# Minys233/GCN-BMP

Hardware: AMD Instinct MI355X
Metric: drug-pairs/sec fwd+bwd, binary-DDI GGNN d=128 (higher is better)
Workload: dtype f32; 1 GPU; C2: full binary DDI set (544 drugs, 147696 pairs), GGNN 4-step d=128 tied + Nie co-attention (head 8, tanh) + MLP(32,16), fwd+bwd+Adam, 1024 pairs/GPU/step, every molecule instance encoded; the 144 batches of one epoch resident in HBM, cycled; layout=per-instance packed layout, whole 128-row tiles, pairs_per_gpu=1024, global_batch=1024, parallelism=dp1

## Files before the change

gcn-bmp_amd/csrc/bmp_fused.hip:

```cpp
#include <type_traits>
#include <string.h>
#include "bmp_kernels.h"

#include "bmp_tile.h"

template <int D, bool FIRST, bool VAR, bool SAVE>
__global__ __launch_bounds__(512) void k_ggnn_step_fwd(StepArgs a) {
    constexpr int LD = D + 4;
    constexpr int NCB = D / 32, NRW = 8 / NCB, RB = 4 / NRW;
    extern __shared__ __attribute__((aligned(16))) float lds[];
    float* Hs = lds;
    float* As = lds + FZ_R * LD;
    float* wds = As + FZ_R * LD;
    int* rptr = (int*)(wds + FZ_R * 4);
    int* ecol = rptr + 132;
    float* evalv = (float*)(ecol + FZ_ECAP);
    int* sy = (int*)(evalv + FZ_ECAP);

    const int tid = threadIdx.x, lane = tid & 63, w = tid >> 6;
    const int grp = w >> 2;
    GrpSync gs{sy + grp, 0};
    if (tid < FZ_NSYNC) sy[tid] = 0;
    if (grp == 0) __builtin_amdgcn_s_setprio(2);
    const int wc = w % NCB, wr = w / NCB;
    const int l31 = lane & 31, hi = lane >> 5;
    FZ_TILE_SETUP();
    if (VAR && a.tile_stride > nrows) {
        const int e = row0 + a.tile_stride;
        fz_clear_rows<512>(a.hout, D, row0 + nrows, e, tid);
        fz_clear_rows<512>(a.m, D, row0 + nrows, e, tid);
        fz_clear_rows<512>(a.rz, 2 * D, row0 + nrows, e, tid);
        fz_clear_rows<512>(a.c, D, row0 + nrows, e, tid);
    }
    const int col = wc * 32 + l31;
    const int wrow0 = wr * RB * 32;
    const int lrow = wrow0 + 4 * hi;
    const int rot = (tile * 8) % D;
    const float* Hw = Hs + (wrow0 + l31) * LD + 4 * hi;
    const float* Aw = As + (wrow0 + l31) * LD + 4 * hi;
    float* Hl = Hs + lrow * LD + col;
    float* Al = As + lrow * LD + col;
#define LOFF(rb, reg) (((rb) * 32 + ((reg) & 3) + 8 * ((reg) >> 2)) * LD)

    constexpr bool save = SAVE;
    for (int idx = tid; idx < nrows * (D / 4); idx += 512) {
        const int r = idx / (D / 4), c4 = idx % (D / 4);
        *(f32x4*)(Hs + r * LD + 4 * c4) = *(const f32x4*)(a.h + (size_t)(row0 + r) * D + 4 * c4);
    }
    const bool csr_lds = stage_csr(a.ptr, a.col, a.val, row0, rptr, ecol, evalv, nrows);
    __syncthreads();
    if (!grp_live) return;
    const RowOrder ro = FZ_ROW_ORDER();
    const int bi = wr & 1;

    auto step = [&](auto first_c, const float* WTs, const float* bEs, const float* ATs, const float* bvs, float* om, float* orz,
                    float* oc, float* oh) {
        constexpr bool FST = decltype(first_c)::value;
        int tmask = 0;
        f32x16 acc_m[1][RB];
        zero_acc(acc_m[0]);
        for (int e = 0; e < 4; ++e) {
            const float* const Bp[1] = {WTs + (size_t)(e * D + 4 * hi) * D + 4 * col};
            const int ldw[1] = {D};
            BPre<1> pre;
            tile_b_prefetch<1>(pre, Bp, ldw, D, rot);
            float wd;
            FZ_GATHER(Hs, As, e, &wd);
            if ((tid & 3) == 0) wds[(tid >> 2) * 4 + e] = wd;
            if (e == 0 && (tid & 3) == 0 && tmask) __hip_atomic_fetch_or(sy + 2 + grp, tmask, __ATOMIC_RELAXED, __HIP_MEMORY_SCOPE_WORKGROUP);
            grp_sync(gs);
            const int any = (__hip_atomic_load(sy + 2 + grp, __ATOMIC_RELAXED, __HIP_MEMORY_SCOPE_WORKGROUP) >> e) & 1;
            if (any) tile_mma_msg<VAR, 1, RB>(nrb, e, ro.nbr, bi, acc_m, Aw, LD, Bp, ldw, D, rot, &pre);
            FZ_GSYNC();
        }
        constexpr int NG = FST ? 2 : 3;
        int ldwg[NG];
    #pragma unroll
        for (int g = 0; g < NG; ++g) ldwg[g] = 3 * D;
        const float* const base_h = ATs + (size_t)(4 * hi) * 3 * D + 4 * col + (FST ? 4 * D : 0);
        const float* const base_m = ATs + (size_t)(D + 4 * hi) * 3 * D + 4 * col + (FST ? 4 * D : 0);
        const float* Bh[NG]; const float* Bm[NG];
    #pragma unroll
        for (int g = 0; g < NG; ++g) { Bh[g] = base_h + 4 * D * g; Bm[g] = base_m + 4 * D * g; }
        BPre<NG> pre_h;
        tile_b_prefetch<NG>(pre_h, (const float* const (&)[NG])Bh, (const int (&)[NG])ldwg, D, rot);
        {
            const AccBuf mo = acc_buf<D>(om, row0, 0, col);
            float be[4];
    #pragma unroll
            for (int e = 0; e < 4; ++e) be[e] = bEs[e * D + col];
            FZ_FOR_ACC {
                const int tp = lrow + rb * 32 + (reg & 3) + 8 * (reg >> 2);
                const int r = (tp & 64) + ro.perm[tp];
                const f32x4 wd4 = *(const f32x4*)(wds + r * 4);
                const float v = __builtin_fmaf(wd4[3], be[3], __builtin_fmaf(wd4[2], be[2], __builtin_fmaf(wd4[1], be[1],
                                               __builtin_fmaf(wd4[0], be[0], acc_m[0][rb][reg]))));
                As[r * LD + col] = v;
                if (save) __builtin_amdgcn_raw_buffer_store_b32(__builtin_bit_cast(unsigned, v), mo.rs, mo.vo + r * D * 4, 0, 0);
            }
        }
        FZ_GSYNC();

        f32x16 acc_g[3][RB];
        zero_acc(acc_g[0]); zero_acc(acc_g[1]); zero_acc(acc_g[2]);
        {
            f32x16 gg[NG][RB];
    #pragma unroll
            for (int g = 0; g < NG; ++g) zero_acc(gg[g]);
            BPre<NG> pre_m;
            tile_b_prefetch<NG>(pre_m, (const float* const (&)[NG])Bm, (const int (&)[NG])ldwg, D, rot);
            tile_mma_n<VAR, NG, RB>(nrb, gg, Hw, LD, (const float* const (&)[NG])Bh, (const int (&)[NG])ldwg, D, rot, &pre_h);
            tile_mma_n<VAR, NG, RB>(nrb, gg, Aw, LD, (const float* const (&)[NG])Bm, (const int (&)[NG])ldwg, D, rot, &pre_m);
    #pragma unroll
            for (int g = 0; g < NG; ++g)
    #pragma unroll
                for (int rb = 0; rb < RB; ++rb) acc_g[g + (FST ? 1 : 0)][rb] = gg[g][rb];
        }
        const float br = bvs[col], bz = bvs[D + col], bcn = bvs[2 * D + col];
        {
            const AccBuf rzo = acc_buf<2 * D>(orz, row0, lrow, col);
            FZ_FOR_ACC {
                const float zv = bmp_sigmoid(acc_g[1][rb][reg] + bz);
                acc_g[1][rb][reg] = zv;
                if (save) acc_st<2 * D>(rzo, rb, reg, zv, D);
                if (!FST) {
                    const float rv = bmp_sigmoid(acc_g[0][rb][reg] + br);
                    acc_g[0][rb][reg] = rv;
                    if (save) acc_st<2 * D>(rzo, rb, reg, rv, 0);
                }
            }
        }
        if (!FST) {
            const float* const Bu[1] = {a.UcT + (size_t)(4 * hi) * D + 4 * col};
            const int ldu[1] = {D};
            BPre<1> pre_u;
            tile_b_prefetch<1>(pre_u, Bu, ldu, D, rot);
            FZ_GSYNC();
            FZ_FOR_ACC { Al[LOFF(rb, reg)] = acc_g[0][rb][reg] * Hl[LOFF(rb, reg)]; }
            FZ_GSYNC();
            f32x16 gc[1][RB];
    #pragma unroll
            for (int rb = 0; rb < RB; ++rb) gc[0][rb] = acc_g[2][rb];
            tile_mma_n<VAR, 1, RB>(nrb, gc, Aw, LD, Bu, ldu, D, rot, &pre_u);
    #pragma unroll
            for (int rb = 0; rb < RB; ++rb) acc_g[2][rb] = gc[0][rb];
        }
        {
            const AccBuf co = acc_buf<D>(oc, row0, lrow, col);
            const AccBuf ho = acc_buf<D>(oh, row0, lrow, col);
            FZ_FOR_ACC {
                const float cv = bmp_tanh(acc_g[2][rb][reg] + bcn);
                const float zv = acc_g[1][rb][reg];
                float hn = zv * cv;
                if (!FST) hn = __builtin_fmaf(1.f - zv, Hl[LOFF(rb, reg)], hn);
                if (save) acc_st<D>(co, rb, reg, cv);
                acc_st<D>(ho, rb, reg, hn);
            }
        }
    };
    step(std::integral_constant<bool, FIRST>{}, a.WT, a.bE, a.AT, a.b, a.m, a.rz, a.c, a.hout);
}

template <int D, bool FIRST, bool VAR>
__global__ __launch_bounds__(512) void k_ggnn_step_bwd(StepArgs a) {
    constexpr int LD = D + 4;
    constexpr int NCB = D / 32, NRW = 8 / NCB, RB = 4 / NRW;
    constexpr int F4 = D / 4;
    constexpr int NV = D / 16;
    extern __shared__ __attribute__((aligned(16))) float lds[];
    float* Xs = lds;
    float* Ys = lds + FZ_R * LD;
    int* rptr = (int*)(Ys + FZ_R * LD + FZ_R * 4);
    int* ecol = rptr + 132;
    float* evalv = (float*)(ecol + FZ_ECAP);
    int* sy = (int*)(evalv + FZ_ECAP);

    const int tid = threadIdx.x, lane = tid & 63, w = tid >> 6;
    const int grp = w >> 2;
    GrpSync gs{sy + grp, 0};
    int tmask = 0;
    if (tid < FZ_NSYNC) sy[tid] = 0;
    if (grp == 0) __builtin_amdgcn_s_setprio(2);
    const int wc = w % NCB, wr = w / NCB;
    const int l31 = lane & 31, hi = lane >> 5;
    FZ_TILE_SETUP();
    if (VAR && a.tile_stride > nrows) {
        const int e = row0 + a.tile_stride;
        fz_clear_rows<512>(a.dh, D, row0 + nrows, e, tid);
        fz_clear_rows<512>(a.gda, 7 * D, row0 + nrows, e, tid);
    }
    const int col = wc * 32 + l31;
    const int wrow0 = wr * RB * 32;
    const int lrow = wrow0 + 4 * hi;
    const int rot = (tile * 8) % D;
    const float* Xw = Xs + (wrow0 + l31) * LD + 4 * hi;
    const float* Yw = Ys + (wrow0 + l31) * LD + 4 * hi;
    float* Xl = Xs + lrow * LD + col;
    float* Yl = Ys + lrow * LD + col;
    constexpr bool first = FIRST;
    const int tg = tid & 255;
#define RM_ROW(v) (grp * 64 + ((v) * 256 + tg) / F4)
#define RM_C4(v) (((v) * 256 + tg) % F4)
#define RM_LDS(T, v) (*(f32x4*)((T) + RM_ROW(v) * LD + 4 * RM_C4(v)))
#define RM_LIVE(v) (!VAR || grp * 64 + (v) * (256 / F4) < nrows)
    const AccBuf b_g = rm_buf<D, D>(a.dhout, row0, grp, tg), b_c = rm_buf<D, D>(a.c, row0, grp, tg);
    const AccBuf b_h = rm_buf<D, D>(a.h, row0, grp, tg), b_rz = rm_buf<D, 2 * D>(a.rz, row0, grp, tg);
    const AccBuf b_o = rm_buf<D, 7 * D>(a.gda, row0, grp, tg), b_dh = rm_buf<D, D>(a.dh, row0, grp, tg);

    const bool csr_lds = stage_csr(a.ptr, a.col, a.val, row0, rptr, ecol, evalv, nrows);
    if (!grp_live) {
        __syncthreads();
        return;
    }

    f32x4 ex[NV];
    {
        const f32x4 one = (f32x4){1.f, 1.f, 1.f, 1.f};
        f32x4 g4[NV], z4[NV], c4[NV], h4[NV];
#pragma unroll
        for (int v = 0; v < NV; ++v) if (RM_LIVE(v)) {
            g4[v] = rm_ld<D, D>(b_g, v);
            z4[v] = rm_ld<D, 2 * D>(b_rz, v, D);
            c4[v] = rm_ld<D, D>(b_c, v);
            if (!first) h4[v] = rm_ld<D, D>(b_h, v);
        }
#pragma unroll
        for (int v = 0; v < NV; ++v) if (RM_LIVE(v)) {
            const f32x4 gz = g4[v] * z4[v];
            const f32x4 dac = gz * (one - c4[v] * c4[v]);
            f32x4 dz = gz * (one - z4[v]);
            if (first) { dz *= c4[v]; ex[v] = (f32x4){0.f, 0.f, 0.f, 0.f}; }
            else { dz *= (c4[v] - h4[v]); ex[v] = g4[v] - gz; }
            RM_LDS(Xs, v) = dac;
            RM_LDS(Ys, v) = dz;
            rm_st<D, 7 * D>(b_o, v, dac, 6 * D);
            rm_st<D, 7 * D>(b_o, v, dz, 5 * D);
        }
    }
    const float* const Ac_h = a.A + (size_t)(2 * D + 4 * hi) * 2 * D + 4 * col;
    const float* const Az_h = a.A + (size_t)(D + 4 * hi) * 2 * D + 4 * col;
    const float* const Ar_h = a.A + (size_t)(4 * hi) * 2 * D + 4 * col;
    const int ld2[2] = {2 * D, 2 * D};
    const float* const Bc[2] = {Ac_h, Ac_h + 4 * D};
    BPre<2> pre_c;
    tile_b_prefetch<2>(pre_c, Bc, ld2, D, rot);
    __syncthreads();
    const RowOrder ro = FZ_ROW_ORDER();
    const int bi = wr & 1;
    int aoff[RB];
#pragma unroll
    for (int rb = 0; rb < RB; ++rb) { const int tp = wrow0 + rb * 32 + l31; aoff[rb] = (((tp & 64) + ro.perm[tp]) - (wrow0 + l31)) * LD; }
#define FZ_ROWOF(rb, reg) ((lrow & 64) + ro.perm[lrow + (rb) * 32 + ((reg) & 3) + 8 * ((reg) >> 2)])

    f32x16 acc_x[2][RB];
    zero_acc(acc_x[0]); zero_acc(acc_x[1]);
    tile_mma_n<VAR, 2, RB>(nrb, acc_x, Xw, LD, Bc, ld2, D, rot, &pre_c, aoff);
    if (!first) {
        f32x16 acc_d[1][RB];
        zero_acc(acc_d[0]);
        {
            const float* const Bu[1] = {a.Uc + (size_t)(4 * hi) * D + 4 * col};
            const int ldu[1] = {D};
            tile_mma_n<VAR, 1, RB>(nrb, acc_d, Xw, LD, Bu, ldu, D, rot, nullptr, aoff);
        }
        FZ_GSYNC();
        FZ_FOR_ACC { Xs[FZ_ROWOF(rb, reg) * LD + col] = acc_d[0][rb][reg]; }
        f32x4 r4[NV], h4[NV];
#pragma unroll
        for (int v = 0; v < NV; ++v) if (RM_LIVE(v)) { r4[v] = rm_ld<D, 2 * D>(b_rz, v); h4[v] = rm_ld<D, D>(b_h, v); }
        FZ_GSYNC();
#pragma unroll
        for (int v = 0; v < NV; ++v) if (RM_LIVE(v)) {
            const f32x4 drh = RM_LDS(Xs, v);
            const f32x4 dr = drh * r4[v];
            const f32x4 dar = dr * h4[v] * ((f32x4){1.f, 1.f, 1.f, 1.f} - r4[v]);
            ex[v] += dr;
            RM_LDS(Xs, v) = dar;
            rm_st<D, 7 * D>(b_o, v, dar, 4 * D);
        }
        FZ_GSYNC();
        {
            const float* const Br[2] = {Ar_h, Ar_h + 4 * D};
            tile_mma_n<VAR, 2, RB>(nrb, acc_x, Xw, LD, Br, ld2, D, rot, nullptr, aoff);
        }
    }
    {
        const float* const Bz[2] = {Az_h, Az_h + 4 * D};
        tile_mma_n<VAR, 2, RB>(nrb, acc_x, Yw, LD, Bz, ld2, D, rot, nullptr, aoff);
    }
    FZ_GSYNC();
    FZ_FOR_ACC { Xs[FZ_ROWOF(rb, reg) * LD + col] = acc_x[1][rb][reg]; }
    __syncthreads();

    f32x16 acc_h[1][RB];
#pragma unroll
    for (int rb = 0; rb < RB; ++rb) acc_h[0][rb] = acc_x[0][rb];
    for (int e = 0; e < 4; ++e) {
        const float* const Bp[1] = {a.Wnat + (size_t)(4 * hi) * 4 * D + 4 * (e * D + col)};
        const int ldw[1] = {4 * D};
        BPre<1> pre;
        tile_b_prefetch<1>(pre, Bp, ldw, D, rot);
        float wd;
        const bool has_e = FZ_GATHER(Xs, Ys, e, &wd);
        if ((tid >> 2) < nrows && (has_e || !a.skip_zero_g)) {
            const int row = tid >> 2, q = tid & 3;
            const float* s = Ys + ((row & 64) + ro.inv[row]) * LD + q * (D / 4);
            float* o = a.gda + (size_t)(row0 + row) * 7 * D + e * D + q * (D / 4);
#pragma unroll
            for (int f = 0; f < D / 16; ++f) *(f32x4*)(o + 4 * f) = *(const f32x4*)(s + 4 * f);
        }
        if (e == 0 && (tid & 3) == 0 && tmask) __hip_atomic_fetch_or(sy + 2 + grp, tmask, __ATOMIC_RELAXED, __HIP_MEMORY_SCOPE_WORKGROUP);
        grp_sync(gs);
        const int any = (__hip_atomic_load(sy + 2 + grp, __ATOMIC_RELAXED, __HIP_MEMORY_SCOPE_WORKGROUP) >> e) & 1;
        if (any) tile_mma_msg<VAR, 1, RB>(nrb, e, ro.nbr, bi, acc_h, Yw, LD, Bp, ldw, D, rot, &pre);
        FZ_GSYNC();
    }
    FZ_FOR_ACC { Ys[FZ_ROWOF(rb, reg) * LD + col] = acc_h[0][rb][reg]; }
    FZ_GSYNC();
#pragma unroll
    for (int v = 0; v < NV; ++v) if (RM_LIVE(v)) rm_st<D, D>(b_dh, v, RM_LDS(Ys, v) + ex[v]);
#undef RM_LIVE
#undef RM_ROW
#undef RM_C4
#undef RM_LDS
#undef FZ_ROWOF
}

struct RelArgs {
    const int* ptr; const int* col; const float* val;
    int tile0;
    int act;
    const int* mt_row0; const int* mt_nblk;
    int mt_rows;
    const float* h;
    const float* WT;
    const float* bE;
    const float* WsT;
    const float* bs;
    float* out;
    float* wdeg;
    const float* dout; const float* y;
    const float* Wnat;
    const float* Ws;
    float* dh;
    float* gda;
    int skip_zero_g;
};

template <int D, bool VAR>
__global__ __launch_bounds__(512) void k_relgcn_layer_fwd(RelArgs a) {
    constexpr int LD = D + 4;
    constexpr int NCB = D / 32, NRW = 8 / NCB, RB = 4 / NRW;
    extern __shared__ __attribute__((aligned(16))) float lds[];
    float* Hs = lds;
    float* As = lds + FZ_R * LD;
    float* wds = As + FZ_R * LD;
    int* rptr = (int*)(wds + FZ_R * 4);
    int* ecol = rptr + 132;
    float* evalv = (float*)(ecol + FZ_ECAP);
    int* sy = (int*)(evalv + FZ_ECAP);

    const int tid = threadIdx.x, lane = tid & 63, w = tid >> 6;
    const int grp = w >> 2;
    GrpSync gs{sy + grp, 0};
    int tmask = 0;
    if (tid < FZ_NSYNC) sy[tid] = 0;
    if (grp == 0) __builtin_amdgcn_s_setprio(2);
    const int wc = w % NCB, wr = w / NCB;
    const int l31 = lane & 31, hi = lane >> 5;
    FZ_TILE_SETUP();
    const int col = wc * 32 + l31;
    const int wrow0 = wr * RB * 32;
    const int lrow = wrow0 + 4 * hi;
    const int rot = (tile * 8) % D;
    const float* Hw = Hs + (wrow0 + l31) * LD + 4 * hi;
    const float* Aw = As + (wrow0 + l31) * LD + 4 * hi;

    for (int idx = tid; idx < nrows * (D / 4); idx += 512) {
        const int r = idx / (D / 4), c4 = idx % (D / 4);
        *(f32x4*)(Hs + r * LD + 4 * c4) = *(const f32x4*)(a.h + (size_t)(row0 + r) * D + 4 * c4);
    }
    const bool csr_lds = stage_csr(a.ptr, a.col, a.val, row0, rptr, ecol, evalv, nrows);
    __syncthreads();
    if (!grp_live) return;
    const RowOrder ro = FZ_ROW_ORDER();
    const int bi = wr & 1;
    int aoff[RB];
#pragma unroll
    for (int rb = 0; rb < RB; ++rb) { const int tp = wrow0 + rb * 32 + l31; aoff[rb] = (((tp & 64) + ro.perm[tp]) - (wrow0 + l31)) * LD; }

    f32x16 acc[1][RB];
    zero_acc(acc[0]);
    const float* const Bs[1] = {a.WsT + (size_t)(4 * hi) * D + 4 * col};
    const int lds_[1] = {D};
    BPre<1> pre_s;
    for (int e = 0; e < 4; ++e) {
        const float* const Bp[1] = {a.WT + (size_t)(e * D + 4 * hi) * D + 4 * col};
        const int ldw[1] = {D};
        BPre<1> pre;
        tile_b_prefetch<1>(pre, Bp, ldw, D, rot);
        if (e == 3) tile_b_prefetch<1>(pre_s, Bs, lds_, D, rot);
        float wd;
        FZ_GATHER(Hs, As, e, &wd);
        if ((tid & 3) == 0) wds[(tid >> 2) * 4 + e] = wd;
        if (e == 0 && (tid & 3) == 0 && tmask) __hip_atomic_fetch_or(sy + 2 + grp, tmask, __ATOMIC_RELAXED, __HIP_MEMORY_SCOPE_WORKGROUP);
        grp_sync(gs);
        const int any = (__hip_atomic_load(sy + 2 + grp, __ATOMIC_RELAXED, __HIP_MEMORY_SCOPE_WORKGROUP) >> e) & 1;
        if (any) tile_mma_msg<VAR, 1, RB>(nrb, e, ro.nbr, bi, acc, Aw, LD, Bp, ldw, D, rot, &pre);
        FZ_GSYNC();
    }
    tile_mma_n<VAR, 1, RB>(nrb, acc, Hw, LD, Bs, lds_, D, rot, &pre_s, aoff);
    {
        const AccBuf oo = acc_buf<D>(a.out, row0, 0, col);
        float be[4];
#pragma unroll
        for (int e = 0; e < 4; ++e) be[e] = a.bE[e * D + col];
        const float bsv = a.bs ? a.bs[col] : 0.f;
        const int act = a.act;
        FZ_FOR_ACC {
            const int tp = lrow + rb * 32 + (reg & 3) + 8 * (reg >> 2);
            const int r = (tp & 64) + ro.perm[tp];
            const f32x4 wd4 = *(const f32x4*)(wds + r * 4);
            const float v = acc[0][rb][reg] + bsv + wd4[0] * be[0] + wd4[1] * be[1] + wd4[2] * be[2] + wd4[3] * be[3];
            __builtin_amdgcn_raw_buffer_store_b32(__builtin_bit_cast(unsigned, bmp_act(act, v)), oo.rs, oo.vo + r * D * 4, 0, 0);
        }
    }
    if (a.wdeg != nullptr && (tid & 255) < 64 && grp * 64 + (tid & 255) < nrows) {
        const int r = grp * 64 + (tid & 255);
        *(f32x4*)(a.wdeg + (size_t)(row0 + r) * 4) = *(const f32x4*)(wds + r * 4);
    }
}

template <int D, bool VAR>
__global__ __launch_bounds__(512) void k_relgcn_layer_bwd(RelArgs a) {
    constexpr int LD = D + 4;
    constexpr int NCB = D / 32, NRW = 8 / NCB, RB = 4 / NRW;
    constexpr int F4 = D / 4;
    constexpr int NV = D / 16;
    extern __shared__ __attribute__((aligned(16))) float lds[];
    float* Xs = lds;
    float* Ys = lds + FZ_R * LD;
    int* rptr = (int*)(Ys + FZ_R * LD + FZ_R * 4);
    int* ecol = rptr + 132;
    float* evalv = (float*)(ecol + FZ_ECAP);
    int* sy = (int*)(evalv + FZ_ECAP);

    const int tid = threadIdx.x, lane = tid & 63, w = tid >> 6;
    const int grp = w >> 2;
    GrpSync gs{sy + grp, 0};
    int tmask = 0;
    if (tid < FZ_NSYNC) sy[tid] = 0;
    if (grp == 0) __builtin_amdgcn_s_setprio(2);
    const int wc = w % NCB, wr = w / NCB;
    const int l31 = lane & 31, hi = lane >> 5;
    FZ_TILE_SETUP();
    const int col = wc * 32 + l31;
    const int wrow0 = wr * RB * 32;
    const int lrow = wrow0 + 4 * hi;
    const int rot = (tile * 8) % D;
    const float* Xw = Xs + (wrow0 + l31) * LD + 4 * hi;
    const float* Yw = Ys + (wrow0 + l31) * LD + 4 * hi;
    float* Yl = Ys + lrow * LD + col;
    const int tg = tid & 255;
#define RM_ROW(v) (grp * 64 + ((v) * 256 + tg) / F4)
#define RM_C4(v) (((v) * 256 + tg) % F4)
#define RM_LDS(T, v) (*(f32x4*)((T) + RM_ROW(v) * LD + 4 * RM_C4(v)))
#define RM_LIVE(v) (!VAR || grp * 64 + (v) * (256 / F4) < nrows)
    const AccBuf b_g = rm_buf<D, D>(a.dout, row0, grp, tg), b_y = rm_buf<D, D>(a.y, row0, grp, tg);
// ... 410 lines not shown
```

gcn-bmp_amd/csrc/bmp_ops.hip:

```cpp
#include <string.h>
#include "bmp_kernels.h"

static inline RGArgs rg_zero() {
    RGArgs a;
    memset(&a, 0, sizeof(a));
    return a;
}

static inline size_t max_sz(size_t a, size_t b) { return a > b ? a : b; }

__global__ void k_dact(const float* __restrict__ dout, int lddo, const float* __restrict__ out, int ldo, int act, int N,
                       int d, float* __restrict__ dpre) {
    const size_t total = (size_t)N * d;
    for (size_t idx = (size_t)blockIdx.x * blockDim.x + threadIdx.x; idx < total; idx += (size_t)gridDim.x * blockDim.x) {
        const int row = (int)(idx / d), c = (int)(idx % d);
        dpre[idx] = dout[(size_t)row * lddo + c] * bmp_dact(act, out[(size_t)row * ldo + c]);
    }
}

__global__ void k_gru_bwd_gates(const float* __restrict__ dhn, const float* __restrict__ h, const float* __restrict__ rz,
                                const float* __restrict__ c, int N, int d, int first, float* __restrict__ da,
                                float* __restrict__ dhacc) {
    const size_t total = (size_t)N * d;
    for (size_t idx = (size_t)blockIdx.x * blockDim.x + threadIdx.x; idx < total; idx += (size_t)gridDim.x * blockDim.x) {
// ... 303 lines not shown
        a.c_out = c; a.ldc = d;
        a.first = 0;
        if ((rc = bmp_launch_rowgemm(a, n_tiles, BMP_EPI_GRU_OUT, st))) return rc;
    }
    return 0;
}

extern "C" size_t bmp_gru_state_bwd_ws_floats(int n_tiles, int d) { return bmp_gru_bwd_ws_floats(n_tiles, d); }

extern "C" int bmp_gru_state_bwd(const float* dsout, const float* hd, const float* m, const float* s, const float* rz,
                                 const float* c, int n_tiles, int d, const float* A, const float* Urz, const float* Uc, float* dhd,
                                 float* dm, float* ds, float* dWT, float* dUrzT, float* dUcT, float* db, float* ws,
                                 size_t ws_floats, hipStream_t st) {
    BMP_REQUIRE(n_tiles > 0 && d > 0 && (d & 7) == 0 && ws_floats >= bmp_gru_state_bwd_ws_floats(n_tiles, d));
    BMP_REQUIRE(dsout && hd && m && s && rz && c && A && Urz && Uc && dhd && dm && ds && dWT && dUrzT && dUcT && db && ws);
    const int N = n_tiles * BMP_R;
    float* da = ws;
    float* dsacc = da + (size_t)N * 3 * d;
    float* slab = dsacc + (size_t)N * d;
    int rc;
    hipLaunchKernelGGL(k_gru_bwd_gates, dim3(ew_blocks((size_t)N * d)), dim3(256), 0, st, dsout, s, rz, c, N, d, 0, da, dsacc);
    BMP_LAUNCH_CHECK();
    {
        RGArgs a = rg_zero();
        a.s[0] = RGSrc{da + 2 * d, nullptr, Uc, 3 * d, 0, d, d};
        a.nsrc = 1; a.Nout = d;
        a.Y = da; a.ldy = 3 * d;
        a.r = rz; a.ldr = 2 * d;
        a.h = s; a.ldh = d;
        a.o1 = dsacc; a.ldo1 = d;
        if ((rc = bmp_launch_rowgemm(a, n_tiles, BMP_EPI_GRU_DRH, st))) return rc;
    }
    {
        RGArgs a = rg_zero();
        a.s[0] = RGSrc{da, nullptr, A, 3 * d, 0, 2 * d, 3 * d};
        a.nsrc = 1; a.Nout = 2 * d;
        a.Y = dhd; a.ldy = d;
        a.split = d;
        a.o1 = dm; a.ldo1 = d;
        if ((rc = bmp_launch_rowgemm(a, n_tiles, BMP_EPI_GENERIC, st))) return rc;
    }
    {
        RGArgs a = rg_zero();
        a.s[0] = RGSrc{da, nullptr, Urz, 3 * d, 0, d, 2 * d};
        a.nsrc = 1; a.Nout = d;
        a.Y = ds; a.ldy = d;
        a.add = dsacc; a.ldadd = d;
        if ((rc = bmp_launch_rowgemm(a, n_tiles, BMP_EPI_GENERIC, st))) return rc;
    }
    {
        WGArgs g{hd, nullptr, d, 0, da, 3 * d, d, 3 * d, N, dWT, 3 * d, 0, db};
        if ((rc = bmp_launch_wgrad(g, slab, st))) return rc;
        WGArgs g2{m, nullptr, d, 0, da, 3 * d, d, 3 * d, N, dWT + (size_t)d * 3 * d, 3 * d, 0};
        if ((rc = bmp_launch_wgrad(g2, slab, st))) return rc;
        WGArgs g3{s, nullptr, d, 0, da, 3 * d, d, 2 * d, N, dUrzT, 2 * d, 0};
        if ((rc = bmp_launch_wgrad(g3, slab, st))) return rc;
        WGArgs g4{rz, s, 2 * d, d, da + 2 * d, 3 * d, d, d, N, dUcT, d, 0};
        if ((rc = bmp_launch_wgrad(g4, slab, st))) return rc;
    }
    return 0;
}

extern "C" int bmp_readout_fwd(const float* h, const float* h0, int n_tiles, int d, int d0, int o, const float* WT,
                               const float* b, int act_j, const float* row_w, const int* mol_row0, const int* mol_nrows,
                               int n_mols, float* ij, float* g, hipStream_t st) {
    BMP_REQUIRE(n_tiles > 0 && d > 0 && (d & 7) == 0 && o > 0 && n_mols > 0);
    BMP_REQUIRE(h0 == nullptr || (d0 > 0 && (d0 & 7) == 0));
    RGArgs a = rg_zero();
    a.s[0] = RGSrc{h, nullptr, WT, d, 0, 2 * o, d};
    a.nsrc = 1;
    if (h0) {
        a.s[1] = RGSrc{h0, nullptr, WT + (size_t)d * 2 * o, d0, 0, 2 * o, d0};
        a.nsrc = 2;
    }
    a.Nout = 2 * o;
    a.Y = ij; a.ldy = 2 * o;
    a.bias = b;
    a.split = o;
    a.act_lo = BMP_ACT_SIGMOID; a.act_hi = act_j;
    int rc = bmp_launch_rowgemm(a, n_tiles, BMP_EPI_GENERIC, st);
    if (rc) return rc;
    hipLaunchKernelGGL(k_readout_segsum, dim3(n_mols), dim3(256), 0, st, ij, o, row_w, mol_row0, mol_nrows, g);
    BMP_LAUNCH_CHECK();
    return 0;
}

extern "C" size_t bmp_readout_bwd_ws_floats(int n_tiles, int d, int d0, int o) {
    const int N = n_tiles * BMP_R;
    size_t slab = max_sz(bmp_wgrad_ws_floats(N, d, 2 * o), d0 > 0 ? bmp_wgrad_ws_floats(N, d0, 2 * o) : 0);
    slab = max_sz(slab, bmp_colsum_ws_floats(N, 2 * o));
    return (size_t)N * 2 * o + slab;
}

extern "C" int bmp_readout_bwd(const float* dg, const float* h, const float* h0, int n_tiles, int d, int d0, int o,
                               const float* Wnat, const float* ij, int act_j, const float* row_w, const int* mol_row0,
                               const int* mol_nrows, int n_mols, float* dh, float* dh0, float* dWT, float* db,
                               int accumulate_w, float* ws, size_t ws_floats, hipStream_t st, hipStream_t st_w) {
    BMP_REQUIRE(n_tiles > 0 && d > 0 && (d & 7) == 0 && o > 0 && (o & 3) == 0 && n_mols > 0);
    if (!h0) d0 = 0;
    BMP_REQUIRE(ws_floats >= bmp_readout_bwd_ws_floats(n_tiles, d, d0, o));
    const int N = n_tiles * BMP_R;
    float* dij = ws;
    float* slab = dij + (size_t)N * 2 * o;
    hipError_t e = hipMemsetAsync(dij, 0, (size_t)N * 2 * o * sizeof(float), st);
    if (e != hipSuccess) return (int)e;
    hipLaunchKernelGGL(k_readout_bwd_rows, dim3(n_mols), dim3(256), 0, st, dg, ij, o, act_j, row_w, mol_row0, mol_nrows, dij);
    BMP_LAUNCH_CHECK();
    int rc;
    const int acc = accumulate_w ? 1 : 0;
    if (!st_w) st_w = st;
    if ((rc = bmp_fork_to(st, st_w))) return rc;
    {
        RGArgs a = rg_zero();
        a.s[0] = RGSrc{dij, nullptr, Wnat, 2 * o, 0, d + d0, 2 * o};
        a.nsrc = 1; a.Nout = d + d0;
        a.Y = dh; a.ldy = d;
        if (h0) { a.split = d; a.o1 = dh0; a.ldo1 = d0; }
        if ((rc = bmp_launch_rowgemm(a, n_tiles, BMP_EPI_GENERIC, st))) return rc;
    }
    {
        WGArgs g{h, nullptr, d, 0, dij, 2 * o, d, 2 * o, N, dWT, 2 * o, acc, db};
        if ((rc = bmp_launch_wgrad(g, slab, st_w))) return rc;
        if (h0) {
            WGArgs g2{h0, nullptr, d0, 0, dij, 2 * o, d0, 2 * o, N, dWT + (size_t)d * 2 * o, 2 * o, acc};
            if ((rc = bmp_launch_wgrad(g2, slab, st_w))) return rc;
        }
    }
    return 0;
}

extern "C" int bmp_linear_fwd(const float* X, int ldx, int n_tiles, int K, int Nout, const float* WT, int ldw,
                              const float* b, int act, float* Y, int ldy, hipStream_t st) {
    RGArgs a = rg_zero();
    a.s[0] = RGSrc{X, nullptr, WT, ldx, 0, ldw, K};
    a.nsrc = 1; a.Nout = Nout; a.Y = Y; a.ldy = ldy; a.bias = b;
    a.act_lo = a.act_hi = act;
    return bmp_launch_rowgemm(a, n_tiles, BMP_EPI_GENERIC, st);
}

extern "C" size_t bmp_wgrad_ws_floats_c(int N, int K, int Nn) {
    return max_sz(bmp_wgrad_ws_floats(N, K, Nn), bmp_colsum_ws_floats(N, Nn));
}

extern "C" int bmp_linear_wgrad(const float* X, int ldx, const float* dY, int ldy, int N, int K, int Nn, float* dWT,
                                float* db, float* ws, size_t ws_floats, hipStream_t st) {
    BMP_REQUIRE(ws_floats >= bmp_wgrad_ws_floats_c(N, K, Nn));
    WGArgs g{X, nullptr, ldx, 0, dY, ldy, K, Nn, N, dWT, Nn, 0};
    int rc = bmp_launch_wgrad(g, ws, st);
    if (rc) return rc;
    if (db) return bmp_launch_colsum(dY, ldy, N, Nn, db, 0, ws, st);
    return 0;
}

extern "C" int bmp_version(void) { return 409; }
extern "C" int bmp_tile_rows(void) { return BMP_R; }
```

gcn-bmp_amd/csrc/bmp_tile.h:

```cpp
#pragma once
#include <stdlib.h>
#include <type_traits>
#include <string.h>
#include "bmp_kernels.h"

#define FZ_R 128

struct StepArgs {
    const int* ptr; const int* col; const float* val;
    int tile0;
    int first;
    const int* mt_row0; const int* mt_nblk;
    int mt_rows;
    const float* h;
    const float* WT;
    const float* bE;
    const float* AT;
    const float* UcT;
    const float* b;
    float* m; float* rz; float* c; float* hout;
    const float* dhout;
    const float* Wnat;
    const float* A;
    const float* Uc;
    float* dh;
    float* gda;
    int skip_zero_g;
    int tile_stride;
};

template <int NT>
__device__ __forceinline__ void fz_clear_rows(float* p, int W, int r_begin, int r_end, int tid) {
    if (p == nullptr) return;
    const int w4 = W >> 2;
    f32x4* q = (f32x4*)(p + (size_t)r_begin * W);
    const int n = (r_end - r_begin) * w4;
    for (int i = tid; i < n; i += NT) q[i] = (f32x4){0.f, 0.f, 0.f, 0.f};
}

template <int NB>
struct BPre { f32x4 b0[NB], b1[NB]; };
template <int NB>
__device__ __forceinline__ void tile_b_prefetch(BPre<NB>& p, const float* const (&Bp)[NB], const int (&ldw)[NB], int K, int rot) {
    int k1 = rot + 8; if (k1 >= K) k1 -= K;
#pragma unroll
    for (int nb = 0; nb < NB; ++nb) {
        p.b0[nb] = *(const f32x4*)(Bp[nb] + (size_t)rot * ldw[nb]);
        p.b1[nb] = *(const f32x4*)(Bp[nb] + (size_t)k1 * ldw[nb]);
    }
}

template <int NB, int RB, int NRB = RB>
__device__ __forceinline__ void tile_mma(f32x16 (&acc)[NB][RB], const float* As_wave, int LD, const float* const (&Bp)[NB],
                                         const int (&ldw)[NB], int K, int rot, const BPre<NB>* pre = nullptr, const int* aoff = nullptr) {
    f32x4 b0[NB], b1[NB], b2[NB];
    int k = rot;
    int k1 = k + 8; if (k1 >= K) k1 -= K;
#pragma unroll
    for (int nb = 0; nb < NB; ++nb) {
        if (pre) { b0[nb] = pre->b0[nb]; b1[nb] = pre->b1[nb]; }
        else {
            b0[nb] = *(const f32x4*)(Bp[nb] + (size_t)k * ldw[nb]);
            b1[nb] = *(const f32x4*)(Bp[nb] + (size_t)k1 * ldw[nb]);
        }
    }
    f32x4 a0[NRB], a1[NRB];
#pragma unroll
    for (int rb = 0; rb < NRB; ++rb) a0[rb] = *(const f32x4*)(As_wave + (aoff ? aoff[rb] : rb * 32 * LD) + k);
    for (int it = 0; it < K; it += 8) {
        int k2 = k1 + 8; if (k2 >= K) k2 -= K;
#pragma unroll
        for (int nb = 0; nb < NB; ++nb) b2[nb] = *(const f32x4*)(Bp[nb] + (size_t)k2 * ldw[nb]);
#pragma unroll
        for (int rb = 0; rb < NRB; ++rb) a1[rb] = *(const f32x4*)(As_wave + (aoff ? aoff[rb] : rb * 32 * LD) + k1);
        __builtin_amdgcn_sched_barrier(0);
#pragma unroll
        for (int t = 0; t < 4; ++t)
#pragma unroll
            for (int rb = 0; rb < NRB; ++rb)
#pragma unroll
                for (int nb = 0; nb < NB; ++nb) acc[nb][rb] = bmp_mfma(a0[rb][t], b0[nb][t], acc[nb][rb]);
        __builtin_amdgcn_sched_barrier(0);
#pragma unroll
        for (int nb = 0; nb < NB; ++nb) { b0[nb] = b1[nb]; b1[nb] = b2[nb]; }
#pragma unroll
        for (int rb = 0; rb < NRB; ++rb) a0[rb] = a1[rb];
        k = k1; k1 = k2;
    }
}

template <bool VAR, int NB, int RB>
__device__ __forceinline__ void tile_mma_n(int nrb, f32x16 (&acc)[NB][RB], const float* As_wave, int LD, const float* const (&Bp)[NB],
                                           const int (&ldw)[NB], int K, int rot, const BPre<NB>* pre = nullptr, const int* aoff = nullptr) {
    if constexpr (!VAR) {
        tile_mma<NB, RB, RB>(acc, As_wave, LD, Bp, ldw, K, rot, pre, aoff);
    } else if constexpr (RB == 1) {
        if (nrb > 0) tile_mma<NB, 1, 1>(acc, As_wave, LD, Bp, ldw, K, rot, pre, aoff);
    } else {
        if (nrb == RB) tile_mma<NB, RB, RB>(acc, As_wave, LD, Bp, ldw, K, rot, pre, aoff);
        else if (nrb > 0) tile_mma<NB, RB, 1>(acc, As_wave, LD, Bp, ldw, K, rot, pre, aoff);
    }
}

template <int N>
__device__ __forceinline__ void zero_acc(f32x16 (&acc)[N]) {
#pragma unroll
    for (int i = 0; i < N; ++i)
#pragma unroll
        for (int r = 0; r < 16; ++r) acc[i][r] = 0.f;
}

template <int D>
__device__ __forceinline__ bool tile_gather(const float* src_tile, float* dst_tile, int LD, const int* ptr, const int* col,
                                            const float* val, int row0, int e, float* wsum, int* tmask, int nrows = FZ_R,
                                            const unsigned char* inv = nullptr) {
    constexpr int F = D / 16;
    const int row = threadIdx.x >> 2, q = threadIdx.x & 3;
    f32x4 acc[F];
#pragma unroll
    for (int f = 0; f < F; ++f) acc[f] = (f32x4){0.f, 0.f, 0.f, 0.f};
    float wd = 0.f;
    bool any = false;
    *wsum = 0.f;
    if (nrows < FZ_R && row >= nrows) return false;
    const int e0 = ptr[row], e1 = ptr[row + 1];
    for (int ed = e0; ed < e1; ++ed) {
        const int cv = col[ed];
        *tmask |= 1 << (cv & 3);
        if ((cv & 3) == e) {
            const float v = val[ed];
            const float* s = src_tile + ((cv >> 2) - row0) * LD + q * (D / 4);
#pragma unroll
            for (int f = 0; f < F; ++f) acc[f] += *(const f32x4*)(s + 4 * f) * v;
            wd += v;
            any = true;
        }
    }
    float* o = dst_tile + (inv ? (row & 64) + inv[row] : row) * LD + q * (D / 4);
#pragma unroll
    for (int f = 0; f < F; ++f) *(f32x4*)(o + 4 * f) = acc[f];
    *wsum = wd;
    return any;
}

#define FZ_ECAP 1024
__device__ __forceinline__ bool stage_csr(const int* ptr, const int* col, const float* val, int row0, int* rptr, int* ecol,
                                          float* evalv, int nrows = FZ_R, int nt = 512) {
    const int ebase = ptr[row0];
    const int ne = ptr[row0 + nrows] - ebase;
    if (ne > FZ_ECAP) return false;
    for (int i = threadIdx.x; i <= nrows; i += nt) rptr[i] = ptr[row0 + i] - ebase;
    for (int i = threadIdx.x; i < ne; i += nt) { ecol[i] = col[ebase + i]; evalv[i] = val[ebase + i]; }
    return true;
}
#define FZ_GATHER(srcT, dstT, e, wdp) (csr_lds ? tile_gather<D>(srcT, dstT, LD, rptr, ecol, evalv, row0, e, wdp, &tmask, nrows, ro.inv) \
                                               : tile_gather<D>(srcT, dstT, LD, a.ptr + row0, a.col, a.val, row0, e, wdp, &tmask, nrows, ro.inv))
#define FZ_ROW_ORDER() fz_row_order(sy, gs, grp, w, lane, csr_lds ? rptr : a.ptr + row0, csr_lds ? ecol : a.col, nrows)

struct GrpSync {
    int* ctr;
    int target;
};
__device__ __forceinline__ void grp_sync(GrpSync& g) {
    g.target += 4;
    __builtin_amdgcn_fence(__ATOMIC_RELEASE, "workgroup", "local");
    if ((threadIdx.x & 63) == 0) __hip_atomic_fetch_add(g.ctr, 1, __ATOMIC_RELAXED, __HIP_MEMORY_SCOPE_WORKGROUP);
    while (__hip_atomic_load(g.ctr, __ATOMIC_RELAXED, __HIP_MEMORY_SCOPE_WORKGROUP) < g.target) __builtin_amdgcn_s_sleep(1);
    __builtin_amdgcn_fence(__ATOMIC_ACQUIRE, "workgroup", "local");
}
#define FZ_NSYNC 72

#define FZ_RARE_TYPES 0x6
struct RowOrder {
    const unsigned char* inv;
    const unsigned char* perm;
    int nbr;
};
__device__ __forceinline__ RowOrder fz_row_order(int* sy, GrpSync& gs, int grp, int w, int lane, const int* ptr_local, const int* col,
                                                 int nrows) {
    unsigned char* inv = (unsigned char*)(sy + 8);
    unsigned char* perm = (unsigned char*)(sy + 40);
    if ((w & 3) == 0) {
        const int r = grp * 64 + lane;
        int m = 0;
        if (r < nrows)
            for (int ed = ptr_local[r]; ed < ptr_local[r + 1]; ++ed) m |= 1 << (col[ed] & 3);
        const bool rare = (m & FZ_RARE_TYPES) != 0;
        const unsigned long long bal = __ballot(rare), lt = (1ull << lane) - 1ull;
        const int nr = __popcll(bal);
        const int pos = rare ? __popcll(bal & lt) : nr + __popcll(~bal & lt);
        inv[r] = (unsigned char)pos;
        perm[grp * 64 + pos] = (unsigned char)lane;
        if (lane == 0) sy[4 + grp] = nr;
    }
    grp_sync(gs);
    return RowOrder{inv, perm, (sy[4 + grp] + 31) >> 5};
}
template <bool VAR, int NB, int RB>
__device__ __forceinline__ void tile_mma_msg(int nrb, int e, int nbr, int bi, f32x16 (&acc)[NB][RB], const float* As_wave, int LD,
                                             const float* const (&Bp)[NB], const int (&ldw)[NB], int K, int rot, const BPre<NB>* pre) {
    const bool rare = (FZ_RARE_TYPES >> e) & 1;
    if constexpr (RB == 1) {
        if (nrb > 0 && (!rare || bi < nbr)) tile_mma<NB, 1, 1>(acc, As_wave, LD, Bp, ldw, K, rot, pre);
    } else {
        const int nb = rare ? (nbr < nrb ? nbr : nrb) : nrb;
        if (nb >= RB) tile_mma<NB, RB, RB>(acc, As_wave, LD, Bp, ldw, K, rot, pre);
        else if (nb > 0) tile_mma<NB, RB, 1>(acc, As_wave, LD, Bp, ldw, K, rot, pre);
    }
}

struct AccBuf {
    __amdgpu_buffer_rsrc_t rs;
    int vo;
};
template <int LDC>
__device__ __forceinline__ AccBuf acc_buf(const float* base, int tile_row0, int lane_row, int col) {
    AccBuf b;
    b.rs = __builtin_amdgcn_make_buffer_rsrc((void*)(base + (size_t)tile_row0 * LDC), 0, 0x7FFFFFFF, 0x00020000);
    b.vo = (lane_row * LDC + col) * 4;
    return b;
}
template <int LDC>
__device__ __forceinline__ float acc_ld(const AccBuf& b, int rb, int reg, int coff = 0) {
    const int so = ((rb * 32 + (reg & 3) + 8 * (reg >> 2)) * LDC + coff) * 4;
    return __builtin_bit_cast(float, __builtin_amdgcn_raw_buffer_load_b32(b.rs, b.vo, so, 0));
}
template <int LDC>
__device__ __forceinline__ void acc_st(const AccBuf& b, int rb, int reg, float v, int coff = 0) {
    const int so = ((rb * 32 + (reg & 3) + 8 * (reg >> 2)) * LDC + coff) * 4;
    __builtin_amdgcn_raw_buffer_store_b32(__builtin_bit_cast(unsigned, v), b.rs, b.vo, so, 0);
}

typedef unsigned u32x4 __attribute__((ext_vector_type(4)));
template <int D, int LDP>
__device__ __forceinline__ AccBuf rm_buf(const float* base, int tile_row0, int grp, int tg) {
    AccBuf b;
    b.rs = __builtin_amdgcn_make_buffer_rsrc((void*)(base + (size_t)tile_row0 * LDP), 0, 0x7FFFFFFF, 0x00020000);
    b.vo = ((grp * 64 + tg / (D / 4)) * LDP + 4 * (tg % (D / 4))) * 4;
    return b;
}
template <int D, int LDP>
__device__ __forceinline__ f32x4 rm_ld(const AccBuf& b, int v, int coff = 0) {
    const int so = (v * (1024 / D) * LDP + coff) * 4;
    return __builtin_bit_cast(f32x4, __builtin_amdgcn_raw_buffer_load_b128(b.rs, b.vo, so, 0));
}
template <int D, int LDP>
__device__ __forceinline__ void rm_st(const AccBuf& b, int v, f32x4 x, int coff = 0) {
    const int so = (v * (1024 / D) * LDP + coff) * 4;
    __builtin_amdgcn_raw_buffer_store_b128(__builtin_bit_cast(u32x4, x), b.rs, b.vo + so, 0, 0);
}

#define FZ_FOR_ACC _Pragma("unroll") for (int rb = 0; rb < RB; ++rb) if (rb < nrb) _Pragma("unroll") for (int reg = 0; reg < 16; ++reg)

template <int D>
__device__ __forceinline__ int fz_live(int nblk, int wr) {
    constexpr int NCB = D / 32, NRW = 8 / NCB, RB = 4 / NRW;
    const int live = nblk - wr * RB;
    return live < 0 ? 0 : (live > RB ? RB : live);
}
#define FZ_TILE_SETUP()                                                          \
    const int tile = blockIdx.x + a.tile0;                                      \
    const int row0 = VAR ? a.mt_row0[tile] : tile * FZ_R;                       \
    const int nblk = VAR ? a.mt_nblk[tile] : 4;                                 \
    const int nrows = VAR ? nblk * 32 : FZ_R;                                   \
    const int nrb = VAR ? fz_live<D>(nblk, wr) : RB;                            \
    const bool grp_live = VAR ? nblk > 2 * grp : true

#define FZ_GSYNC() grp_sync(gs)
```

Measured before the change: 403,300 pairs/s.

## Interleave gda gradient stores with message MFMA loop and spill ex through dh

The per-edge-type copy of the gathered gradient tile from LDS to global gda now happens inside the MFMA K-loop. A side lambda issues one buffer store per iteration, and sched_group_barrier interleaves those stores with the MFMAs instead of running them as a separate phase before the matmul. To save registers, the ex accumulator is no longer held across the edge-type loop: the partial dh is written to global early and reloaded before the final sum. This aims to hide store latency and lower VGPR pressure, but it adds an extra global write and read of dh and depends on the compiler honoring the scheduling hints.

New measurement: 405,800 pairs/s, median of 6. No clear change (+0.6%).

```diff
diff --git a/gcn-bmp_amd/csrc/bmp_fused.hip b/gcn-bmp_amd/csrc/bmp_fused.hip
--- a/gcn-bmp_amd/csrc/bmp_fused.hip
+++ b/gcn-bmp_amd/csrc/bmp_fused.hip
@@ -161,6 +161,19 @@
     step(std::integral_constant<bool, FIRST>{}, a.WT, a.bE, a.AT, a.b, a.m, a.rz, a.c, a.hout);
 }
 
+template <bool VAR>
+__device__ __forceinline__ f32x4 fz_ex_plus_dr(f32x4 ex, f32x4 drh, f32x4 r, f32x4 dr) {
+    f32x4 o;
+    if constexpr (VAR) {
+#pragma unroll
+        for (int t = 0; t < 4; ++t) o[t] = __builtin_fmaf(drh[t], r[t], ex[t]);
+    } else {
+#pragma clang fp contract(off)
+        o = ex + dr;
+    }
+    return o;
+}
+
 template <int D, bool FIRST, bool VAR>
 __global__ __launch_bounds__(512) void k_ggnn_step_bwd(StepArgs a) {
     constexpr int LD = D + 4;
@@ -229,7 +242,7 @@
             const f32x4 gz = g4[v] * z4[v];
             const f32x4 dac = gz * (one - c4[v] * c4[v]);
             f32x4 dz = gz * (one - z4[v]);
-            if (first) { dz *= c4[v]; ex[v] = (f32x4){0.f, 0.f, 0.f, 0.f}; }
+            if (first) dz *= c4[v];
             else { dz *= (c4[v] - h4[v]); ex[v] = g4[v] - gz; }
             RM_LDS(Xs, v) = dac;
             RM_LDS(Ys, v) = dz;
@@ -274,7 +287,7 @@
             const f32x4 drh = RM_LDS(Xs, v);
             const f32x4 dr = drh * r4[v];
             const f32x4 dar = dr * h4[v] * ((f32x4){1.f, 1.f, 1.f, 1.f} - r4[v]);
-            ex[v] += dr;
+            rm_st<D, D>(b_dh, v, fz_ex_plus_dr<VAR>(ex[v], drh, r4[v], dr));
             RM_LDS(Xs, v) = dar;
             rm_st<D, 7 * D>(b_o, v, dar, 4 * D);
         }
@@ -292,6 +305,7 @@
     FZ_FOR_ACC { Xs[FZ_ROWOF(rb, reg) * LD + col] = acc_x[1][rb][reg]; }
     __syncthreads();
 
+    const __amdgpu_buffer_rsrc_t g_rs = __builtin_amdgcn_make_buffer_rsrc((void*)(a.gda + (size_t)row0 * 7 * D), 0, nrows * 7 * D * 4, 0x00020000);
     f32x16 acc_h[1][RB];
 #pragma unroll
     for (int rb = 0; rb < RB; ++rb) acc_h[0][rb] = acc_x[0][rb];
@@ -302,18 +316,35 @@
         tile_b_prefetch<1>(pre, Bp, ldw, D, rot);
         float wd;
         const bool has_e = FZ_GATHER(Xs, Ys, e, &wd);
-        if ((tid >> 2) < nrows && (has_e || !a.skip_zero_g)) {
-            const int row = tid >> 2, q = tid & 3;
-            const float* s = Ys + ((row & 64) + ro.inv[row]) * LD + q * (D / 4);
-            float* o = a.gda + (size_t)(row0 + row) * 7 * D + e * D + q * (D / 4);
-#pragma unroll
-            for (int f = 0; f < D / 16; ++f) *(f32x4*)(o + 4 * f) = *(const f32x4*)(s + 4 * f);
-        }
+        const bool g_st = (tid >> 2) < nrows && (has_e || !a.skip_zero_g);
+        const int g_row = tid >> 2, g_q = tid & 3;
+        const float* g_s = Ys + ((g_row & 64) + ro.inv[g_row]) * LD + g_q * (D / 4);
         if (e == 0 && (tid & 3) == 0 && tmask) __hip_atomic_fetch_or(sy + 2 + grp, tmask, __ATOMIC_RELAXED, __HIP_MEMORY_SCOPE_WORKGROUP);
         grp_sync(gs);
         const int any = (__hip_atomic_load(sy + 2 + grp, __ATOMIC_RELAXED, __HIP_MEMORY_SCOPE_WORKGROUP) >> e) & 1;
-        if (any) tile_mma_msg<VAR, 1, RB>(nrb, e, ro.nbr, bi, acc_h, Yw, LD, Bp, ldw, D, rot, &pre);
+        bool stored = false;
+        if (any) {
+            const int g_vo = g_st ? (g_row * 7 * D + e * D + g_q * (D / 4)) * 4 : (int)0x80000000u;
+            f32x4 g_cur = *(const f32x4*)g_s;
+            auto g_side = [&](int i, auto) {
+                if (i < D / 16) {
+                    __builtin_amdgcn_raw_buffer_store_b128(__builtin_bit_cast(u32x4, g_cur), g_rs, g_vo + 16 * i, 0, 0);
+                    if (i + 1 < D / 16) g_cur = *(const f32x4*)(g_s + 4 * (i + 1));
+                }
+            };
+            stored = tile_mma_msg_side<VAR, D, 2, 1, RB>(nrb, e, ro.nbr, bi, acc_h, Yw, LD, Bp, ldw, rot, &pre, g_side);
+        }
+        if (!stored && g_st) {
+            float* o = a.gda + (size_t)(row0 + g_row) * 7 * D + e * D + g_q * (D / 4);
+#pragma unroll
+            for (int f = 0; f < D / 16; ++f) *(f32x4*)(o + 4 * f) = *(const f32x4*)(g_s + 4 * f);
+        }
         FZ_GSYNC();
+    }
+#pragma unroll
+    for (int v = 0; v < NV; ++v) {
+        ex[v] = (f32x4){0.f, 0.f, 0.f, 0.f};
+        if (!first && RM_LIVE(v)) ex[v] = rm_ld<D, D>(b_dh, v);
     }
     FZ_FOR_ACC { Ys[FZ_ROWOF(rb, reg) * LD + col] = acc_h[0][rb][reg]; }
     FZ_GSYNC();
diff --git a/gcn-bmp_amd/csrc/bmp_ops.hip b/gcn-bmp_amd/csrc/bmp_ops.hip
--- a/gcn-bmp_amd/csrc/bmp_ops.hip
+++ b/gcn-bmp_amd/csrc/bmp_ops.hip
@@ -479,5 +479,5 @@
     return 0;
 }
 
-extern "C" int bmp_version(void) { return 409; }
+extern "C" int bmp_version(void) { return 410; }
 extern "C" int bmp_tile_rows(void) { return BMP_R; }
diff --git a/gcn-bmp_amd/csrc/bmp_tile.h b/gcn-bmp_amd/csrc/bmp_tile.h
--- a/gcn-bmp_amd/csrc/bmp_tile.h
+++ b/gcn-bmp_amd/csrc/bmp_tile.h
@@ -89,6 +89,57 @@
     }
 }
 
+#define FZ_SG_MFMA 0x008
+#define FZ_SG_VMEM_READ 0x020
+#define FZ_SG_DS_READ 0x100
+#define FZ_SG_SIDE (0x002 | 0x004 | 0x040 | 0x080 | 0x400)
+template <int NB, int RB, int NRB, int K, int SPM, class Side>
+__device__ __forceinline__ void tile_mma_side(f32x16 (&acc)[NB][RB], const float* As_wave, int LD, const float* const (&Bp)[NB],
+                                              const int (&ldw)[NB], int rot, const BPre<NB>* pre, const int* aoff, Side& side) {
+    f32x4 b0[NB], b1[NB], b2[NB];
+    int k = rot;
+    int k1 = k + 8; if (k1 >= K) k1 -= K;
+#pragma unroll
+    for (int nb = 0; nb < NB; ++nb) {
+        if (pre) { b0[nb] = pre->b0[nb]; b1[nb] = pre->b1[nb]; }
+        else {
+            b0[nb] = *(const f32x4*)(Bp[nb] + (size_t)k * ldw[nb]);
+            b1[nb] = *(const f32x4*)(Bp[nb] + (size_t)k1 * ldw[nb]);
+        }
+    }
+    f32x4 a0[NRB], a1[NRB];
+#pragma unroll
+    for (int rb = 0; rb < NRB; ++rb) a0[rb] = *(const f32x4*)(As_wave + (aoff ? aoff[rb] : rb * 32 * LD) + k);
+    __builtin_amdgcn_sched_barrier(0);
+#pragma unroll
+    for (int i = 0; i < K / 8; ++i) {
+        int k2 = k1 + 8; if (k2 >= K) k2 -= K;
+#pragma unroll
+        for (int nb = 0; nb < NB; ++nb) b2[nb] = *(const f32x4*)(Bp[nb] + (size_t)k2 * ldw[nb]);
+#pragma unroll
+        for (int rb = 0; rb < NRB; ++rb) a1[rb] = *(const f32x4*)(As_wave + (aoff ? aoff[rb] : rb * 32 * LD) + k1);
+        side(i, std::integral_constant<int, NRB>{});
+#pragma unroll
+        for (int t = 0; t < 4; ++t)
+#pragma unroll
+            for (int rb = 0; rb < NRB; ++rb)
+#pragma unroll
+                for (int nb = 0; nb < NB; ++nb) acc[nb][rb] = bmp_mfma(a0[rb][t], b0[nb][t], acc[nb][rb]);
+        __builtin_amdgcn_sched_group_barrier(FZ_SG_VMEM_READ, NB, 0);
+        __builtin_amdgcn_sched_group_barrier(FZ_SG_DS_READ, NRB, 0);
+#pragma unroll
+        for (int q = 0; q < 4 * NRB * NB; ++q) {
+            __builtin_amdgcn_sched_group_barrier(FZ_SG_MFMA, 1, 0);
+            __builtin_amdgcn_sched_group_barrier(FZ_SG_SIDE, SPM, 0);
+        }
+        __builtin_amdgcn_sched_barrier(0);
+#pragma unroll
+        for (int nb = 0; nb < NB; ++nb) { b0[nb] = b1[nb]; b1[nb] = b2[nb]; }
+#pragma unroll
+        for (int rb = 0; rb < NRB; ++rb) a0[rb] = a1[rb];
+        k = k1; k1 = k2;
+    }
+}
 template <bool VAR, int NB, int RB>
 __device__ __forceinline__ void tile_mma_n(int nrb, f32x16 (&acc)[NB][RB], const float* As_wave, int LD, const float* const (&Bp)[NB],
                                            const int (&ldw)[NB], int K, int rot, const BPre<NB>* pre = nullptr, const int* aoff = nullptr) {
@@ -209,6 +260,20 @@
     }
 }
 
+template <bool VAR, int K, int SPM, int NB, int RB, class Side>
+__device__ __forceinline__ bool tile_mma_msg_side(int nrb, int e, int nbr, int bi, f32x16 (&acc)[NB][RB], const float* As_wave, int LD,
+                                                  const float* const (&Bp)[NB], const int (&ldw)[NB], int rot, const BPre<NB>* pre, Side& side) {
+    const bool rare = (FZ_RARE_TYPES >> e) & 1;
+    if constexpr (RB == 1) {
+        if (nrb > 0 && (!rare || bi < nbr)) { tile_mma_side<NB, 1, 1, K, SPM>(acc, As_wave, LD, Bp, ldw, rot, pre, nullptr, side); return true; }
+    } else {
+        const int nb = rare ? (nbr < nrb ? nbr : nrb) : nrb;
+        if (nb >= RB) { tile_mma_side<NB, RB, RB, K, SPM>(acc, As_wave, LD, Bp, ldw, rot, pre, nullptr, side); return true; }
+        else if (nb > 0) { tile_mma_side<NB, RB, 1, K, SPM>(acc, As_wave, LD, Bp, ldw, rot, pre, nullptr, side); return true; }
+    }
+    return false;
+}
+
 struct AccBuf {
     __amdgpu_buffer_rsrc_t rs;
     int vo;
```
